# nvidia-cosmos/cosmos-curate

Measured on NVIDIA H100. Metric: clips_per_sec, higher is better.
Workload: dtype f16

## Files before the change

### cosmos_curate_b200/csrc/gemm.cu

```cuda
#include <cuda_fp16.h>

#include <algorithm>
#include <cstdlib>

#include "common.h"
#include "ptx.cuh"

namespace cb {

constexpr int BM = 128, BK = 64;
constexpr int kGemmThreads = 384;
constexpr int kEpiRows = 64, kEpiBytes = kEpiRows * 128;

template <int BN>
struct GemmCfg {
  static constexpr int kStages = (BN == 256) ? 4 : 6;
  static constexpr int kABytes = BM * BK * 2, kBBytes = BN * BK * 2;
  static constexpr int kStageBytes = kABytes + kBBytes;
  static constexpr int kRingBytes = kStages * kStageBytes;
  static constexpr int kEpiTotal = 2  * 2  * kEpiBytes;
  static constexpr int kSmem = kRingBytes + kEpiTotal + 1024  + 256 ;
  static_assert(kSmem <= 232448, "over the 227 KB of opt-in shared memory per block on sm_90");
};

struct GemmArgs {
  const float* bias;
  int M, N, K;
  int residual;
};

__device__ __forceinline__ float act_quick_gelu(float x) { return __fdividef(x, 1.f + exp2f(-2.4554669595930156f * x)); }
__device__ __forceinline__ float act_gelu_tanh(float x) {
  const float k0 = 0.7978845608028654f, k1 = 0.044715f;
  const float u = k0 * (x + k1 * x * x * x);
  const float e = exp2f(2.885390081777927f * u);
  const float t = 1.f - __fdividef(2.f, e + 1.f);
  return 0.5f * x * (1.f + t);
}

template <int ACT>
__device__ __forceinline__ float act(float x) {
  if (ACT == CB_EPI_QUICK_GELU) return act_quick_gelu(x);
  if (ACT == CB_EPI_GELU_TANH) return act_gelu_tanh(x);
  return x;
}

template <int BN>
__device__ __forceinline__ void wgmma_tile(float* d, uint64_t da, uint64_t db, int accumulate) {
  if (BN == 256) wgmma_m64n256k16(d, da, db, accumulate);
  else wgmma_m64n128k16(d, da, db, accumulate);
}

template <int BN, int ACT, bool OUT_F32>
__global__ void __launch_bounds__(kGemmThreads, 1)
    gemm_wgmma_kernel(const __grid_constant__ CUtensorMap map_a, const __grid_constant__ CUtensorMap map_b, const __grid_constant__ CUtensorMap map_o,
                      const __grid_constant__ CUtensorMap map_r, const GemmArgs g) {
  using Cfg = GemmCfg<BN>;
  constexpr int kSliceCols = OUT_F32 ? 32 : 64;
  constexpr int kSlices = BN / kSliceCols;
  constexpr int kSliceJ = kSliceCols / 8;
  extern __shared__ __align__(1024) uint8_t smem_raw[];
  const uint32_t base = (smem_u32(smem_raw) + 1023u) & ~1023u;
  uint8_t* smem = smem_raw + (base - smem_u32(smem_raw));
  uint8_t* sA = smem;
  uint8_t* sB = smem + Cfg::kStages * Cfg::kABytes;
  uint8_t* sE = smem + Cfg::kRingBytes;
  uint64_t* full = (uint64_t*)(smem + Cfg::kRingBytes + Cfg::kEpiTotal);
  uint64_t* empty = full + Cfg::kStages;
  uint64_t* rfull = empty + Cfg::kStages;

  const int warp = threadIdx.x >> 5, lane = threadIdx.x & 31, wg = warp >> 2;
  const int m_tiles = (g.M + BM - 1) / BM, n_tiles = (g.N + BN - 1) / BN;
  const int num_tiles = m_tiles * n_tiles;
  const int num_kb = (g.K + BK - 1) / BK;
  const int first = blockIdx.x, step = gridDim.x;
  const bool has_res = OUT_F32 && g.residual;

  if (threadIdx.x == 0) {
    tma_prefetch_desc(&map_a);
    tma_prefetch_desc(&map_b);
    tma_prefetch_desc(&map_o);
    if (has_res) tma_prefetch_desc(&map_r);
    for (int i = 0; i < Cfg::kStages; ++i) {
      mbar_init(&full[i], 1);
      mbar_init(&empty[i], 2);
    }
    for (int i = 0; i < 4; ++i) mbar_init(&rfull[i], 1);
    fence_barrier_init();
  }
  __syncthreads();

  if (wg == 0) {
    reg_dealloc<40>();
    if (warp == 0 && lane == 0) {
      int stage = 0;
      uint32_t phase = 0;
      for (int t = first; t < num_tiles; t += step) {
        const int m_blk = t / n_tiles, n_blk = t % n_tiles;
        if (has_res)
          for (int r = 0; r < BM; r += kEpiRows)
            for (int cc = 0; cc < BN && n_blk * BN + cc < g.N; cc += kSliceCols) tma_prefetch_l2_2d(&map_r, n_blk * BN + cc, m_blk * BM + r);
        for (int kb = 0; kb < num_kb; ++kb) {
          mbar_wait(&empty[stage], phase ^ 1);
          mbar_expect_tx(&full[stage], Cfg::kStageBytes);
          tma_load_2d(sA + stage * Cfg::kABytes, &map_a, &full[stage], kb * BK, m_blk * BM);
          tma_load_2d(sB + stage * Cfg::kBBytes, &map_b, &full[stage], kb * BK, n_blk * BN);
          if (++stage == Cfg::kStages) stage = 0, phase ^= 1;
        }
      }
    }
  } else {
    reg_alloc<232>();
    const int c = wg - 1;
    const bool leader = (threadIdx.x & 127) == 0;
    auto release = [&](int s) {
      if (leader) mbar_arrive(&empty[s]);
    };
    uint8_t* ebuf = sE + c * 2 * kEpiBytes;
    uint64_t* rbar = rfull + 2 * c;
    int eb = 0;
    uint32_t rphase = 0;
    int stage = 0;
    uint32_t phase = 0;
    float acc[BN / 2];
    float2 bias[BN / 8];
    for (int t = first; t < num_tiles; t += step) {
      const int m_blk = t / n_tiles, n_blk = t % n_tiles;
      const int row0 = m_blk * BM + c * 64, col0 = n_blk * BN;
      const int nslices = row0 >= g.M ? 0 : std::min(kSlices, (g.N - col0 + kSliceCols - 1) / kSliceCols);
      int prev = -1;
      for (int kb = 0; kb < num_kb; ++kb) {
        mbar_wait(&full[stage], phase);
        const uint64_t da = wgmma_desc_sw128(smem_u32(sA + stage * Cfg::kABytes + c * (64 * 128)));
        const uint64_t db = wgmma_desc_sw128(smem_u32(sB + stage * Cfg::kBBytes));
        wgmma_fence();
#pragma unroll
        for (int k = 0; k < BK / 16; ++k) wgmma_tile<BN>(acc, da + (uint64_t)(2 * k), db + (uint64_t)(2 * k), (kb | k) != 0);
        wgmma_commit();
        if (kb == 0 && has_res && leader) {
          bulk_wait_read<0>();
          for (int s = 0; s < 2 && s < nslices; ++s) {
            const int b = eb ^ s;
            mbar_expect_tx(&rbar[b], kEpiBytes);
            tma_load_2d(ebuf + b * kEpiBytes, &map_r, &rbar[b], col0 + s * kSliceCols, row0);
          }
        }
        wgmma_wait<1>();
        if (prev >= 0) release(prev);
        prev = stage;
        if (++stage == Cfg::kStages) stage = 0, phase ^= 1;
      }
#pragma unroll
      for (int j = 0; j < BN / 8; ++j) {
        const int col = col0 + 8 * j + 2 * (lane & 3);
        bias[j] = (g.bias && col < g.N) ? __ldg((const float2*)(g.bias + col)) : make_float2(0.f, 0.f);
      }
      wgmma_wait<0>();
      release(prev);

      const int rl = (warp & 3) * 16 + (lane >> 2), sw = lane >> 2;
#pragma unroll
      for (int s = 0; s < kSlices; ++s) {
        if (s >= nslices) break;
        uint8_t* buf = ebuf + eb * kEpiBytes;
        if (has_res) {
          mbar_wait(&rbar[eb], (rphase >> eb) & 1);
          rphase ^= 1u << eb;
        } else {
          if (leader) bulk_wait_read<1>();
          named_bar_sync(1 + c, 128);
        }
#pragma unroll
        for (int jj = 0; jj < kSliceJ; ++jj) {
          const int j = s * kSliceJ + jj;
#pragma unroll
          for (int h = 0; h < 2; ++h) {
            uint8_t* row = buf + (rl + 8 * h) * 128;
            float v0 = act<ACT>(acc[4 * j + 2 * h] + bias[j].x), v1 = act<ACT>(acc[4 * j + 2 * h + 1] + bias[j].y);
            if (OUT_F32) {
              float2* p = (float2*)(row + (((2 * jj + ((lane & 3) >> 1)) ^ sw) << 4) + 8 * (lane & 1));
              if (has_res) {
                const float2 rr = *p;
                v0 += rr.x, v1 += rr.y;
              }
              *p = make_float2(v0, v1);
            } else {
              *(__half2*)(row + ((jj ^ sw) << 4) + 4 * (lane & 3)) = __floats2half2_rn(v0, v1);
            }
          }
        }
        fence_proxy_async();
        named_bar_sync(1 + c, 128);
        if (leader) {
          tma_store_2d(&map_o, buf, col0 + s * kSliceCols, row0);
          bulk_commit();
          if (has_res && s + 2 < nslices) {
            bulk_wait_read<0>();
            mbar_expect_tx(&rbar[eb], kEpiBytes);
            tma_load_2d(buf, &map_r, &rbar[eb], col0 + (s + 2) * kSliceCols, row0);
          }
        }
        eb ^= 1;
      }
    }
    if (leader) bulk_wait<0>();
  }
}

template <int BN, int ACT, bool OUT_F32>
static int launch_gemm(cb_ctx* ctx, const CUtensorMap& ma, const CUtensorMap& mb, const CUtensorMap& mo, const CUtensorMap& mr, const GemmArgs& g,
                       cudaStream_t stream) {
  using Cfg = GemmCfg<BN>;
  auto kern = gemm_wgmma_kernel<BN, ACT, OUT_F32>;
  static bool attr_done[64] = {};
  bool& attr_set = attr_done[ctx->device & 63];
  if (!attr_set) {
    CB_CUDA(ctx, cudaFuncSetAttribute(kern, cudaFuncAttributeMaxDynamicSharedMemorySize, Cfg::kSmem));
    attr_set = true;
  }
  const int tiles = ((g.M + BM - 1) / BM) * ((g.N + BN - 1) / BN);
  mark_launch(ctx, CB_PROF_GEMM, stream);
  kern<<<std::min(tiles, ctx->sm_count), kGemmThreads, Cfg::kSmem, stream>>>(ma, mb, mo, mr, g);
  CB_CUDA(ctx, cudaGetLastError());
  return CB_OK;
}

template <int BN>
static int dispatch_gemm(cb_ctx* ctx, const CUtensorMap& ma, const CUtensorMap& mb, const CUtensorMap& mo, const CUtensorMap& mr, const GemmArgs& g,
                         bool out_f32, int epilogue, cudaStream_t stream) {
  if (out_f32) return launch_gemm<BN, CB_EPI_NONE, true>(ctx, ma, mb, mo, mr, g, stream);
  if (epilogue == CB_EPI_QUICK_GELU) return launch_gemm<BN, CB_EPI_QUICK_GELU, false>(ctx, ma, mb, mo, mr, g, stream);
  if (epilogue == CB_EPI_GELU_TANH) return launch_gemm<BN, CB_EPI_GELU_TANH, false>(ctx, ma, mb, mo, mr, g, stream);
  if (epilogue == CB_EPI_NONE) return launch_gemm<BN, CB_EPI_NONE, false>(ctx, ma, mb, mo, mr, g, stream);
  return fail(ctx, CB_ERR_ARG, "gemm: unknown epilogue %d", epilogue);
}

int gemm_f16(cb_ctx* ctx, const void* A, const void* W, const float* bias, const float* residual, float* out_f32, void* out_f16, int M,
             int N, int K, int epilogue, cudaStream_t stream) {
  if (!A || !W || (!out_f32 && !out_f16)) return fail(ctx, CB_ERR_ARG, "gemm: null operand");
  if (M <= 0 || N <= 0 || K <= 0) return fail(ctx, CB_ERR_ARG, "gemm: bad shape %dx%dx%d", M, N, K);
  if ((K & 7) || (N & 7)) return fail(ctx, CB_ERR_ARG, "gemm: N and K must be multiples of 8 (got N=%d K=%d)", N, K);
  if (((uintptr_t)A | (uintptr_t)W) & 15) return fail(ctx, CB_ERR_ARG, "gemm: operands must be 16-byte aligned");
  const void* out = out_f32 ? (const void*)out_f32 : out_f16;
  if (((uintptr_t)out | (uintptr_t)residual) & 15) return fail(ctx, CB_ERR_ARG, "gemm: output and residual must be 16-byte aligned");
  if (out_f32 && epilogue != CB_EPI_NONE) return fail(ctx, CB_ERR_UNSUPPORTED, "gemm: activation with fp32 output");
  if (residual && !out_f32) return fail(ctx, CB_ERR_UNSUPPORTED, "gemm: residual needs the fp32 output");
  const int tiles256 = ((M + BM - 1) / BM) * ((N + 255) / 256);
  const bool wide = (N % 256 == 0 || N > 1024) && tiles256 >= ctx->sm_count;
  const int BN = wide ? 256 : 128;
  CUtensorMap ma, mb, mo, mr;
  uint64_t da[2] = {(uint64_t)K, (uint64_t)M}, db[2] = {(uint64_t)K, (uint64_t)N}, st[1] = {(uint64_t)K * 2};
  uint32_t ba[2] = {BK, BM}, bb[2] = {BK, (uint32_t)BN};
  int rc = make_tensor_map(ctx, &ma, CU_TENSOR_MAP_DATA_TYPE_FLOAT16, 2, A, da, st, ba, CU_TENSOR_MAP_SWIZZLE_128B);
  if (rc) return rc;
  rc = make_tensor_map(ctx, &mb, CU_TENSOR_MAP_DATA_TYPE_FLOAT16, 2, W, db, st, bb, CU_TENSOR_MAP_SWIZZLE_128B);
  if (rc) return rc;
  const uint64_t esz = out_f32 ? 4 : 2;
  uint64_t dout[2] = {(uint64_t)N, (uint64_t)M}, sout[1] = {(uint64_t)N * esz};
  uint32_t bout[2] = {(uint32_t)(128 / esz), (uint32_t)kEpiRows};
  const CUtensorMapDataType dt = out_f32 ? CU_TENSOR_MAP_DATA_TYPE_FLOAT32 : CU_TENSOR_MAP_DATA_TYPE_FLOAT16;
  rc = make_tensor_map(ctx, &mo, dt, 2, out, dout, sout, bout, CU_TENSOR_MAP_SWIZZLE_128B);
  if (rc) return rc;
  mr = mo;
  if (residual && (rc = make_tensor_map(ctx, &mr, dt, 2, residual, dout, sout, bout, CU_TENSOR_MAP_SWIZZLE_128B))) return rc;
  GemmArgs g{bias, M, N, K, residual != nullptr};
  return BN == 256 ? dispatch_gemm<256>(ctx, ma, mb, mo, mr, g, out_f32 != nullptr, epilogue, stream)
                   : dispatch_gemm<128>(ctx, ma, mb, mo, mr, g, out_f32 != nullptr, epilogue, stream);
}

}

extern "C" int cb_gemm_f16(cb_ctx* ctx, const void* A, const void* W, const float* bias, const float* residual, float* out_f32,
                           void* out_f16, int M, int N, int K, int epilogue, void* stream) {
  if (!ctx) return CB_ERR_ARG;
  return cb::gemm_f16(ctx, A, W, bias, residual, out_f32, out_f16, M, N, K, epilogue, (cudaStream_t)stream);
}
```

### cosmos_curate_b200/csrc/ptx.cuh

```cuda
#pragma once
#include <cuda.h>
#include <cuda_fp16.h>
#include <stdint.h>

namespace cb {

__device__ __forceinline__ uint32_t smem_u32(const void* p) { return (uint32_t)__cvta_generic_to_shared(p); }

__device__ __forceinline__ void mbar_init(uint64_t* bar, uint32_t count) {
  asm volatile("mbarrier.init.shared::cta.b64 [%0], %1;" ::"r"(smem_u32(bar)), "r"(count));
}
__device__ __forceinline__ void fence_barrier_init() { asm volatile("fence.mbarrier_init.release.cluster;" ::: "memory"); }
__device__ __forceinline__ void fence_proxy_async() { asm volatile("fence.proxy.async.shared::cta;" ::: "memory"); }
__device__ __forceinline__ void mbar_expect_tx(uint64_t* bar, uint32_t bytes) {
  asm volatile("mbarrier.arrive.expect_tx.shared::cta.b64 _, [%0], %1;" ::"r"(smem_u32(bar)), "r"(bytes) : "memory");
}
__device__ __forceinline__ void mbar_arrive(uint64_t* bar) {
  asm volatile("mbarrier.arrive.shared::cta.b64 _, [%0];" ::"r"(smem_u32(bar)) : "memory");
}
__device__ __forceinline__ bool mbar_try_wait(uint64_t* bar, uint32_t parity) {
  uint32_t ok;
  asm volatile(
      "{\n\t.reg .pred p;\n\t"
      "mbarrier.try_wait.parity.shared::cta.b64 p, [%1], %2;\n\t"
      "selp.u32 %0, 1, 0, p;\n\t}"
      : "=r"(ok)
      : "r"(smem_u32(bar)), "r"(parity)
      : "memory");
  return ok != 0;
}
__device__ __forceinline__ void mbar_wait(uint64_t* bar, uint32_t parity) {
  while (!mbar_try_wait(bar, parity)) {
  }
}
__device__ __forceinline__ bool mbar_test(uint64_t* bar, uint32_t parity) {
  uint32_t ok;
  asm volatile(
      "{\n\t.reg .pred p;\n\t"
      "mbarrier.test_wait.parity.shared::cta.b64 p, [%1], %2;\n\t"
      "selp.u32 %0, 1, 0, p;\n\t}"
      : "=r"(ok)
      : "r"(smem_u32(bar)), "r"(parity)
      : "memory");
  return ok != 0;
}
__device__ __forceinline__ void mbar_wait_parked(uint64_t* bar, uint32_t parity, uint32_t ns = 20000) {
  uint32_t ok;
  do {
    asm volatile(
        "{\n\t.reg .pred p;\n\t"
        "mbarrier.try_wait.parity.shared::cta.b64 p, [%1], %2, %3;\n\t"
        "selp.u32 %0, 1, 0, p;\n\t}"
        : "=r"(ok)
        : "r"(smem_u32(bar)), "r"(parity), "r"(ns)
        : "memory");
  } while (!ok);
}

__device__ __forceinline__ void tma_prefetch_desc(const CUtensorMap* m) {
  asm volatile("prefetch.tensormap [%0];" ::"l"(m) : "memory");
}
__device__ __forceinline__ void tma_load_2d(void* dst, const CUtensorMap* m, uint64_t* bar, int c0, int c1) {
  asm volatile(
      "cp.async.bulk.tensor.2d.shared::cluster.global.mbarrier::complete_tx::bytes [%0], [%1, {%3, %4}], [%2];" ::"r"(smem_u32(dst)),
      "l"(m), "r"(smem_u32(bar)), "r"(c0), "r"(c1)
      : "memory");
}
__device__ __forceinline__ void tma_load_3d(void* dst, const CUtensorMap* m, uint64_t* bar, int c0, int c1, int c2) {
  asm volatile(
      "cp.async.bulk.tensor.3d.shared::cluster.global.mbarrier::complete_tx::bytes [%0], [%1, {%3, %4, %5}], [%2];" ::"r"(
          smem_u32(dst)),
      "l"(m), "r"(smem_u32(bar)), "r"(c0), "r"(c1), "r"(c2)
      : "memory");
}
__device__ __forceinline__ void tma_load_2d_hint(void* dst, const CUtensorMap* m, uint64_t* bar, int c0, int c1, uint64_t policy) {
  asm volatile(
      "cp.async.bulk.tensor.2d.shared::cluster.global.mbarrier::complete_tx::bytes.L2::cache_hint [%0], [%1, {%3, %4}], [%2], %5;" ::"r"(
          smem_u32(dst)),
      "l"(m), "r"(smem_u32(bar)), "r"(c0), "r"(c1), "l"(policy)
      : "memory");
}
__device__ __forceinline__ void tma_prefetch_l2_2d(const CUtensorMap* m, int c0, int c1) {
  asm volatile("cp.async.bulk.prefetch.tensor.2d.L2.global.tile [%0, {%1, %2}];" ::"l"(m), "r"(c0), "r"(c1) : "memory");
}

__device__ __forceinline__ void tma_store_2d(const CUtensorMap* m, const void* src, int c0, int c1) {
  asm volatile("cp.async.bulk.tensor.2d.global.shared::cta.bulk_group [%0, {%2, %3}], [%1];" ::"l"(m), "r"(smem_u32(src)), "r"(c0), "r"(c1)
               : "memory");
}
__device__ __forceinline__ void bulk_commit() { asm volatile("cp.async.bulk.commit_group;" ::: "memory"); }
template <int N>
__device__ __forceinline__ void bulk_wait_read() {
  asm volatile("cp.async.bulk.wait_group.read %0;" ::"n"(N) : "memory");
}
template <int N>
__device__ __forceinline__ void bulk_wait() {
  asm volatile("cp.async.bulk.wait_group %0;" ::"n"(N) : "memory");
}
__device__ __forceinline__ void named_bar_sync(int id, int threads) { asm volatile("bar.sync %0, %1;" ::"r"(id), "r"(threads) : "memory"); }

__device__ __forceinline__ uint64_t policy_evict_first() {
  uint64_t p;
  asm volatile("createpolicy.fractional.L2::evict_first.b64 %0, 1.0;" : "=l"(p));
  return p;
}
__device__ __forceinline__ uint64_t policy_evict_last() {
  uint64_t p;
  asm volatile("createpolicy.fractional.L2::evict_last.b64 %0, 1.0;" : "=l"(p));
  return p;
}
__device__ __forceinline__ void wgmma_fence() { asm volatile("wgmma.fence.sync.aligned;" ::: "memory"); }
__device__ __forceinline__ void wgmma_commit() { asm volatile("wgmma.commit_group.sync.aligned;" ::: "memory"); }
template <int N>
__device__ __forceinline__ void wgmma_wait() {
  asm volatile("wgmma.wait_group.sync.aligned %0;" ::"n"(N) : "memory");
}
template <int REGS>
__device__ __forceinline__ void reg_alloc() { asm volatile("setmaxnreg.inc.sync.aligned.u32 %0;" ::"n"(REGS)); }
template <int REGS>
__device__ __forceinline__ void reg_dealloc() { asm volatile("setmaxnreg.dec.sync.aligned.u32 %0;" ::"n"(REGS)); }

__device__ __forceinline__ uint64_t wgmma_desc_sw128(uint32_t smem_addr) {
  return (uint64_t)((smem_addr & 0x3FFFF) >> 4) | ((uint64_t)1 << 16) | ((uint64_t)(1024 >> 4) << 32) | ((uint64_t)1 << 62);
}
__device__ __forceinline__ uint64_t wgmma_desc_sw128_mn(uint32_t smem_addr) {
  return (uint64_t)((smem_addr & 0x3FFFF) >> 4) | ((uint64_t)(1024 >> 4) << 16) | ((uint64_t)(1024 >> 4) << 32) | ((uint64_t)1 << 62);
}

__device__ __forceinline__ void wgmma_m64n8k16(float* d, uint64_t desc_a, uint64_t desc_b, int accumulate) {
  asm volatile(
      "{\n\t.reg .pred p;\n\tsetp.ne.b32 p, %6, 0;\n\t"
      "wgmma.mma_async.sync.aligned.m64n8k16.f32.f16.f16 {%0, %1, %2, %3}, %4, %5, p, 1, 1, 0, 0;\n\t}"
      :
        "+f"(d[0]), "+f"(d[1]), "+f"(d[2]), "+f"(d[3])
      : "l"(desc_a), "l"(desc_b), "r"(accumulate));
}
__device__ __forceinline__ void wgmma_m64n32k16(float* d, uint64_t desc_a, uint64_t desc_b, int accumulate) {
  asm volatile(
      "{\n\t.reg .pred p;\n\tsetp.ne.b32 p, %18, 0;\n\t"
      "wgmma.mma_async.sync.aligned.m64n32k16.f32.f16.f16 {%0, %1, %2, %3, %4, %5, %6, %7, %8, %9, %10, %11, %12, %13, %14, %15}, %16, %17, p, 1, 1, 0, 0;\n\t}"
      :
        "+f"(d[0]), "+f"(d[1]), "+f"(d[2]), "+f"(d[3]), "+f"(d[4]), "+f"(d[5]), "+f"(d[6]), "+f"(d[7]),
        "+f"(d[8]), "+f"(d[9]), "+f"(d[10]), "+f"(d[11]), "+f"(d[12]), "+f"(d[13]), "+f"(d[14]), "+f"(d[15])
      : "l"(desc_a), "l"(desc_b), "r"(accumulate));
}
__device__ __forceinline__ void wgmma_m64n128k16(float* d, uint64_t desc_a, uint64_t desc_b, int accumulate) {
  asm volatile(
      "{\n\t.reg .pred p;\n\tsetp.ne.b32 p, %66, 0;\n\t"
      "wgmma.mma_async.sync.aligned.m64n128k16.f32.f16.f16 {%0, %1, %2, %3, %4, %5, %6, %7, %8, %9, %10, %11, %12, %13, %14, %15, %16, %17, %18, %19, %20, %21, %22, %23, %24, %25, %26, %27, %28, %29, %30, %31, %32, %33, %34, %35, %36, %37, %38, %39, %40, %41, %42, %43, %44, %45, %46, %47, %48, %49, %50, %51, %52, %53, %54, %55, %56, %57, %58, %59, %60, %61, %62, %63}, %64, %65, p, 1, 1, 0, 0;\n\t}"
      :
        "+f"(d[0]), "+f"(d[1]), "+f"(d[2]), "+f"(d[3]), "+f"(d[4]), "+f"(d[5]), "+f"(d[6]), "+f"(d[7]),
        "+f"(d[8]), "+f"(d[9]), "+f"(d[10]), "+f"(d[11]), "+f"(d[12]), "+f"(d[13]), "+f"(d[14]), "+f"(d[15]),
        "+f"(d[16]), "+f"(d[17]), "+f"(d[18]), "+f"(d[19]), "+f"(d[20]), "+f"(d[21]), "+f"(d[22]), "+f"(d[23]),
        "+f"(d[24]), "+f"(d[25]), "+f"(d[26]), "+f"(d[27]), "+f"(d[28]), "+f"(d[29]), "+f"(d[30]), "+f"(d[31]),
        "+f"(d[32]), "+f"(d[33]), "+f"(d[34]), "+f"(d[35]), "+f"(d[36]), "+f"(d[37]), "+f"(d[38]), "+f"(d[39]),
        "+f"(d[40]), "+f"(d[41]), "+f"(d[42]), "+f"(d[43]), "+f"(d[44]), "+f"(d[45]), "+f"(d[46]), "+f"(d[47]),
        "+f"(d[48]), "+f"(d[49]), "+f"(d[50]), "+f"(d[51]), "+f"(d[52]), "+f"(d[53]), "+f"(d[54]), "+f"(d[55]),
        "+f"(d[56]), "+f"(d[57]), "+f"(d[58]), "+f"(d[59]), "+f"(d[60]), "+f"(d[61]), "+f"(d[62]), "+f"(d[63])
      : "l"(desc_a), "l"(desc_b), "r"(accumulate));
}
__device__ __forceinline__ void wgmma_m64n256k16(float* d, uint64_t desc_a, uint64_t desc_b, int accumulate) {
  asm volatile(
      "{\n\t.reg .pred p;\n\tsetp.ne.b32 p, %130, 0;\n\t"
      "wgmma.mma_async.sync.aligned.m64n256k16.f32.f16.f16 {%0, %1, %2, %3, %4, %5, %6, %7, %8, %9, %10, %11, %12, %13, %14, %15, %16, %17, %18, %19, %20, %21, %22, %23, %24, %25, %26, %27, %28, %29, %30, %31, %32, %33, %34, %35, %36, %37, %38, %39, %40, %41, %42, %43, %44, %45, %46, %47, %48, %49, %50, %51, %52, %53, %54, %55, %56, %57, %58, %59, %60, %61, %62, %63, %64, %65, %66, %67, %68, %69, %70, %71, %72, %73, %74, %75, %76, %77, %78, %79, %80, %81, %82, %83, %84, %85, %86, %87, %88, %89, %90, %91, %92, %93, %94, %95, %96, %97, %98, %99, %100, %101, %102, %103, %104, %105, %106, %107, %108, %109, %110, %111, %112, %113, %114, %115, %116, %117, %118, %119, %120, %121, %122, %123, %124, %125, %126, %127}, %128, %129, p, 1, 1, 0, 0;\n\t}"
      :
        "+f"(d[0]), "+f"(d[1]), "+f"(d[2]), "+f"(d[3]), "+f"(d[4]), "+f"(d[5]), "+f"(d[6]), "+f"(d[7]),
        "+f"(d[8]), "+f"(d[9]), "+f"(d[10]), "+f"(d[11]), "+f"(d[12]), "+f"(d[13]), "+f"(d[14]), "+f"(d[15]),
        "+f"(d[16]), "+f"(d[17]), "+f"(d[18]), "+f"(d[19]), "+f"(d[20]), "+f"(d[21]), "+f"(d[22]), "+f"(d[23]),
        "+f"(d[24]), "+f"(d[25]), "+f"(d[26]), "+f"(d[27]), "+f"(d[28]), "+f"(d[29]), "+f"(d[30]), "+f"(d[31]),
        "+f"(d[32]), "+f"(d[33]), "+f"(d[34]), "+f"(d[35]), "+f"(d[36]), "+f"(d[37]), "+f"(d[38]), "+f"(d[39]),
        "+f"(d[40]), "+f"(d[41]), "+f"(d[42]), "+f"(d[43]), "+f"(d[44]), "+f"(d[45]), "+f"(d[46]), "+f"(d[47]),
        "+f"(d[48]), "+f"(d[49]), "+f"(d[50]), "+f"(d[51]), "+f"(d[52]), "+f"(d[53]), "+f"(d[54]), "+f"(d[55]),
        "+f"(d[56]), "+f"(d[57]), "+f"(d[58]), "+f"(d[59]), "+f"(d[60]), "+f"(d[61]), "+f"(d[62]), "+f"(d[63]),
        "+f"(d[64]), "+f"(d[65]), "+f"(d[66]), "+f"(d[67]), "+f"(d[68]), "+f"(d[69]), "+f"(d[70]), "+f"(d[71]),
        "+f"(d[72]), "+f"(d[73]), "+f"(d[74]), "+f"(d[75]), "+f"(d[76]), "+f"(d[77]), "+f"(d[78]), "+f"(d[79]),
        "+f"(d[80]), "+f"(d[81]), "+f"(d[82]), "+f"(d[83]), "+f"(d[84]), "+f"(d[85]), "+f"(d[86]), "+f"(d[87]),
        "+f"(d[88]), "+f"(d[89]), "+f"(d[90]), "+f"(d[91]), "+f"(d[92]), "+f"(d[93]), "+f"(d[94]), "+f"(d[95]),
        "+f"(d[96]), "+f"(d[97]), "+f"(d[98]), "+f"(d[99]), "+f"(d[100]), "+f"(d[101]), "+f"(d[102]), "+f"(d[103]),
        "+f"(d[104]), "+f"(d[105]), "+f"(d[106]), "+f"(d[107]), "+f"(d[108]), "+f"(d[109]), "+f"(d[110]), "+f"(d[111]),
        "+f"(d[112]), "+f"(d[113]), "+f"(d[114]), "+f"(d[115]), "+f"(d[116]), "+f"(d[117]), "+f"(d[118]), "+f"(d[119]),
        "+f"(d[120]), "+f"(d[121]), "+f"(d[122]), "+f"(d[123]), "+f"(d[124]), "+f"(d[125]), "+f"(d[126]), "+f"(d[127])
      : "l"(desc_a), "l"(desc_b), "r"(accumulate));
}
__device__ __forceinline__ void wgmma_m64n64k16_ra_tb(float* d, const uint32_t* a, uint64_t desc_b, int accumulate) {
  asm volatile(
      "{\n\t.reg .pred p;\n\tsetp.ne.b32 p, %37, 0;\n\t"
      "wgmma.mma_async.sync.aligned.m64n64k16.f32.f16.f16 {%0, %1, %2, %3, %4, %5, %6, %7, %8, %9, %10, %11, %12, %13, %14, %15, %16, %17, %18, %19, %20, %21, %22, %23, %24, %25, %26, %27, %28, %29, %30, %31}, {%32, %33, %34, %35}, %36, p, 1, 1, 1;\n\t}"
      :
        "+f"(d[0]), "+f"(d[1]), "+f"(d[2]), "+f"(d[3]), "+f"(d[4]), "+f"(d[5]), "+f"(d[6]), "+f"(d[7]),
        "+f"(d[8]), "+f"(d[9]), "+f"(d[10]), "+f"(d[11]), "+f"(d[12]), "+f"(d[13]), "+f"(d[14]), "+f"(d[15]),
        "+f"(d[16]), "+f"(d[17]), "+f"(d[18]), "+f"(d[19]), "+f"(d[20]), "+f"(d[21]), "+f"(d[22]), "+f"(d[23]),
        "+f"(d[24]), "+f"(d[25]), "+f"(d[26]), "+f"(d[27]), "+f"(d[28]), "+f"(d[29]), "+f"(d[30]), "+f"(d[31])
      : "r"(a[0]), "r"(a[1]), "r"(a[2]), "r"(a[3]), "l"(desc_b), "r"(accumulate));
}

__device__ __forceinline__ uint32_t cluster_ctarank() {
  uint32_t r;
  asm volatile("mov.u32 %0, %%cluster_ctarank;" : "=r"(r));
  return r;
}
__device__ __forceinline__ void cluster_sync_all() {
  asm volatile("barrier.cluster.arrive.release.aligned;" ::: "memory");
  asm volatile("barrier.cluster.wait.acquire.aligned;" ::: "memory");
}
__device__ __forceinline__ void mbar_arrive_cluster(uint32_t addr) {
  asm volatile("mbarrier.arrive.release.cluster.shared::cluster.b64 _, [%0];" ::"r"(addr) : "memory");
}
__device__ __forceinline__ uint32_t map_to_cta(const void* local, uint32_t rank) {
  uint32_t r;
  asm volatile("mapa.shared::cluster.u32 %0, %1, %2;" : "=r"(r) : "r"(smem_u32(local)), "r"(rank));
  return r;
}

}
```

Measured before the change: 250.8.

## Add ping-pong warpgroup GEMM schedule for large tiles with heavy epilogues

Adds a ping-pong mode where each consumer warpgroup computes a whole 128x128 tile and the two warpgroups alternate tiles. Named barriers hand off the mainloop turn so one group's epilogue (activation or residual add) overlaps the other's MMAs. It is chosen for large GEMMs with N divisible by 256 that carry an activation or residual. The residual L2 prefetch moves from the producer to the consumer leaders, and the stage count is now derived from the shared-memory limit. Each ping-pong warpgroup holds twice as many accumulator registers, which raises register pressure, and the barrier handoff ordering is delicate.

Result: faster. 258.1, median of 6 (+2.9%).

```diff
diff --git a/cosmos_curate_b200/csrc/gemm.cu b/cosmos_curate_b200/csrc/gemm.cu
--- a/cosmos_curate_b200/csrc/gemm.cu
+++ b/cosmos_curate_b200/csrc/gemm.cu
@@ -8,19 +8,22 @@
 
 namespace cb {
 
-constexpr int BM = 128, BK = 64;
+constexpr int BK = 64;
 constexpr int kGemmThreads = 384;
 constexpr int kEpiRows = 64, kEpiBytes = kEpiRows * 128;
+constexpr int kSmemLimit = 232448;
+constexpr int BM = 128;
+constexpr int kBarTurn = 3;
 
 template <int BN>
 struct GemmCfg {
-  static constexpr int kStages = (BN == 256) ? 4 : 6;
   static constexpr int kABytes = BM * BK * 2, kBBytes = BN * BK * 2;
   static constexpr int kStageBytes = kABytes + kBBytes;
+  static constexpr int kEpiTotal = 2  * 2  * kEpiBytes;
+  static constexpr int kStages = std::min(6, (kSmemLimit - kEpiTotal - 1024 - 256) / kStageBytes);
   static constexpr int kRingBytes = kStages * kStageBytes;
-  static constexpr int kEpiTotal = 2  * 2  * kEpiBytes;
   static constexpr int kSmem = kRingBytes + kEpiTotal + 1024  + 256 ;
-  static_assert(kSmem <= 232448, "over the 227 KB of opt-in shared memory per block on sm_90");
+  static_assert(kSmem <= kSmemLimit, "over the opt-in shared memory per block");
 };
 
 struct GemmArgs {
@@ -51,11 +54,14 @@
   else wgmma_m64n128k16(d, da, db, accumulate);
 }
 
-template <int BN, int ACT, bool OUT_F32>
+template <int WM, int BN, bool PP, int ACT, bool OUT_F32>
 __global__ void __launch_bounds__(kGemmThreads, 1)
     gemm_wgmma_kernel(const __grid_constant__ CUtensorMap map_a, const __grid_constant__ CUtensorMap map_b, const __grid_constant__ CUtensorMap map_o,
                       const __grid_constant__ CUtensorMap map_r, const GemmArgs g) {
   using Cfg = GemmCfg<BN>;
+  static_assert(WM * (PP ? 1 : 2) == BM, "a ping-pong warpgroup computes the whole tile, a cooperative one half of it");
+  constexpr int kBlocks = WM / 64;
+  constexpr int kAcc = BN / 2;
   constexpr int kSliceCols = OUT_F32 ? 32 : 64;
   constexpr int kSlices = BN / kSliceCols;
   constexpr int kSliceJ = kSliceCols / 8;
@@ -83,7 +89,7 @@
     if (has_res) tma_prefetch_desc(&map_r);
     for (int i = 0; i < Cfg::kStages; ++i) {
       mbar_init(&full[i], 1);
-      mbar_init(&empty[i], 2);
+      mbar_init(&empty[i], PP ? 1 : 2);
     }
     for (int i = 0; i < 4; ++i) mbar_init(&rfull[i], 1);
     fence_barrier_init();
@@ -97,9 +103,6 @@
       uint32_t phase = 0;
       for (int t = first; t < num_tiles; t += step) {
         const int m_blk = t / n_tiles, n_blk = t % n_tiles;
-        if (has_res)
-          for (int r = 0; r < BM; r += kEpiRows)
-            for (int cc = 0; cc < BN && n_blk * BN + cc < g.N; cc += kSliceCols) tma_prefetch_l2_2d(&map_r, n_blk * BN + cc, m_blk * BM + r);
         for (int kb = 0; kb < num_kb; ++kb) {
           mbar_wait(&empty[stage], phase ^ 1);
           mbar_expect_tx(&full[stage], Cfg::kStageBytes);
@@ -120,30 +123,43 @@
     uint64_t* rbar = rfull + 2 * c;
     int eb = 0;
     uint32_t rphase = 0;
-    int stage = 0;
-    uint32_t phase = 0;
-    float acc[BN / 2];
+    float acc[kBlocks * kAcc];
     float2 bias[BN / 8];
-    for (int t = first; t < num_tiles; t += step) {
+    constexpr int kTileStep = PP ? 2 : 1;
+    for (int i = PP ? c : 0, t = first + i * step; t < num_tiles; i += kTileStep, t += kTileStep * step) {
       const int m_blk = t / n_tiles, n_blk = t % n_tiles;
-      const int row0 = m_blk * BM + c * 64, col0 = n_blk * BN;
-      const int nslices = row0 >= g.M ? 0 : std::min(kSlices, (g.N - col0 + kSliceCols - 1) / kSliceCols);
+      const int row_in_tile = PP ? 0 : c * WM;
+      const int row0 = m_blk * BM + row_in_tile, col0 = n_blk * BN;
+      const int nb = row0 >= g.M ? 0 : std::min(kBlocks, (g.M - row0 + 63) / 64);
+      const int ns = std::min(kSlices, (g.N - col0 + kSliceCols - 1) / kSliceCols);
+      const int nq = nb * ns;
+      auto load_residual = [&](int q, int b) {
+        const int blk = q / ns;
+        mbar_expect_tx(&rbar[b], kEpiBytes);
+        tma_load_2d(ebuf + b * kEpiBytes, &map_r, &rbar[b], col0 + (q - blk * ns) * kSliceCols, row0 + 64 * blk);
+      };
+      if (has_res && leader)
+        for (int q = 0; q < nq; ++q) tma_prefetch_l2_2d(&map_r, col0 + (q % ns) * kSliceCols, row0 + 64 * (q / ns));
+
+      int stage = (i * num_kb) % Cfg::kStages;
+      uint32_t phase = ((i * num_kb) / Cfg::kStages) & 1;
+      if (PP && i > 0) named_bar_sync(kBarTurn + c, 256);
       int prev = -1;
       for (int kb = 0; kb < num_kb; ++kb) {
         mbar_wait(&full[stage], phase);
-        const uint64_t da = wgmma_desc_sw128(smem_u32(sA + stage * Cfg::kABytes + c * (64 * 128)));
+        const uint64_t da = wgmma_desc_sw128(smem_u32(sA + stage * Cfg::kABytes + row_in_tile * 128));
         const uint64_t db = wgmma_desc_sw128(smem_u32(sB + stage * Cfg::kBBytes));
         wgmma_fence();
 #pragma unroll
-        for (int k = 0; k < BK / 16; ++k) wgmma_tile<BN>(acc, da + (uint64_t)(2 * k), db + (uint64_t)(2 * k), (kb | k) != 0);
+        for (int k = 0; k < BK / 16; ++k)
+#pragma unroll
+          for (int blk = 0; blk < kBlocks; ++blk)
+            wgmma_tile<BN>(acc + blk * kAcc, da + (uint64_t)(blk * (64 * 128 >> 4) + 2 * k), db + (uint64_t)(2 * k), (kb | k) != 0);
         wgmma_commit();
+        if (PP && kb == num_kb - 1 && t + step < num_tiles) named_bar_arrive(kBarTurn + (c ^ 1), 256);
         if (kb == 0 && has_res && leader) {
           bulk_wait_read<0>();
-          for (int s = 0; s < 2 && s < nslices; ++s) {
-            const int b = eb ^ s;
-            mbar_expect_tx(&rbar[b], kEpiBytes);
-            tma_load_2d(ebuf + b * kEpiBytes, &map_r, &rbar[b], col0 + s * kSliceCols, row0);
-          }
+          for (int q = 0; q < 2 && q < nq; ++q) load_residual(q, eb ^ q);
         }
         wgmma_wait<1>();
         if (prev >= 0) release(prev);
@@ -159,59 +175,64 @@
       release(prev);
 
       const int rl = (warp & 3) * 16 + (lane >> 2), sw = lane >> 2;
-#pragma unroll
-      for (int s = 0; s < kSlices; ++s) {
-        if (s >= nslices) break;
-        uint8_t* buf = ebuf + eb * kEpiBytes;
-        if (has_res) {
-          mbar_wait(&rbar[eb], (rphase >> eb) & 1);
-          rphase ^= 1u << eb;
-        } else {
-          if (leader) bulk_wait_read<1>();
-          named_bar_sync(1 + c, 128);
-        }
-#pragma unroll
-        for (int jj = 0; jj < kSliceJ; ++jj) {
-          const int j = s * kSliceJ + jj;
-#pragma unroll
-          for (int h = 0; h < 2; ++h) {
-            uint8_t* row = buf + (rl + 8 * h) * 128;
-            float v0 = act<ACT>(acc[4 * j + 2 * h] + bias[j].x), v1 = act<ACT>(acc[4 * j + 2 * h + 1] + bias[j].y);
-            if (OUT_F32) {
-              float2* p = (float2*)(row + (((2 * jj + ((lane & 3) >> 1)) ^ sw) << 4) + 8 * (lane & 1));
-              if (has_res) {
-                const float2 rr = *p;
-                v0 += rr.x, v1 += rr.y;
+      int q = 0;
+#pragma unroll
+      for (int blk = 0; blk < kBlocks; ++blk) {
+#pragma unroll
+        for (int s = 0; s < kSlices; ++s) {
+          if (blk >= nb || s >= ns) break;
+          uint8_t* buf = ebuf + eb * kEpiBytes;
+          if (has_res) {
+            mbar_wait(&rbar[eb], (rphase >> eb) & 1);
+            rphase ^= 1u << eb;
+          } else {
+            if (leader) bulk_wait_read<1>();
+            named_bar_sync(1 + c, 128);
+          }
+#pragma unroll
+          for (int jj = 0; jj < kSliceJ; ++jj) {
+            const int j = s * kSliceJ + jj;
+            const float* a = acc + blk * kAcc + 4 * j;
+#pragma unroll
+            for (int h = 0; h < 2; ++h) {
+              uint8_t* row = buf + (rl + 8 * h) * 128;
+              float v0 = act<ACT>(a[2 * h] + bias[j].x), v1 = act<ACT>(a[2 * h + 1] + bias[j].y);
+              if (OUT_F32) {
+                float2* p = (float2*)(row + (((2 * jj + ((lane & 3) >> 1)) ^ sw) << 4) + 8 * (lane & 1));
+                if (has_res) {
+                  const float2 rr = *p;
+                  v0 += rr.x, v1 += rr.y;
+                }
+                *p = make_float2(v0, v1);
+              } else {
+                *(__half2*)(row + ((jj ^ sw) << 4) + 4 * (lane & 3)) = __floats2half2_rn(v0, v1);
               }
-              *p = make_float2(v0, v1);
-            } else {
-              *(__half2*)(row + ((jj ^ sw) << 4) + 4 * (lane & 3)) = __floats2half2_rn(v0, v1);
             }
           }
+          fence_proxy_async();
+          named_bar_sync(1 + c, 128);
+          if (leader) {
+            tma_store_2d(&map_o, buf, col0 + s * kSliceCols, row0 + 64 * blk);
+            bulk_commit();
+            if (has_res && q + 2 < nq) {
+              bulk_wait_read<0>();
+              load_residual(q + 2, eb);
+            }
+          }
+          eb ^= 1;
+          ++q;
         }
-        fence_proxy_async();
-        named_bar_sync(1 + c, 128);
-        if (leader) {
-          tma_store_2d(&map_o, buf, col0 + s * kSliceCols, row0);
-          bulk_commit();
-          if (has_res && s + 2 < nslices) {
-            bulk_wait_read<0>();
-            mbar_expect_tx(&rbar[eb], kEpiBytes);
-            tma_load_2d(buf, &map_r, &rbar[eb], col0 + (s + 2) * kSliceCols, row0);
-          }
-        }
-        eb ^= 1;
       }
     }
     if (leader) bulk_wait<0>();
   }
 }
 
-template <int BN, int ACT, bool OUT_F32>
+template <int WM, int BN, bool PP, int ACT, bool OUT_F32>
 static int launch_gemm(cb_ctx* ctx, const CUtensorMap& ma, const CUtensorMap& mb, const CUtensorMap& mo, const CUtensorMap& mr, const GemmArgs& g,
                        cudaStream_t stream) {
   using Cfg = GemmCfg<BN>;
-  auto kern = gemm_wgmma_kernel<BN, ACT, OUT_F32>;
+  auto kern = gemm_wgmma_kernel<WM, BN, PP, ACT, OUT_F32>;
   static bool attr_done[64] = {};
   bool& attr_set = attr_done[ctx->device & 63];
   if (!attr_set) {
@@ -225,13 +246,13 @@
   return CB_OK;
 }
 
-template <int BN>
+template <int WM, int BN, bool PP>
 static int dispatch_gemm(cb_ctx* ctx, const CUtensorMap& ma, const CUtensorMap& mb, const CUtensorMap& mo, const CUtensorMap& mr, const GemmArgs& g,
                          bool out_f32, int epilogue, cudaStream_t stream) {
-  if (out_f32) return launch_gemm<BN, CB_EPI_NONE, true>(ctx, ma, mb, mo, mr, g, stream);
-  if (epilogue == CB_EPI_QUICK_GELU) return launch_gemm<BN, CB_EPI_QUICK_GELU, false>(ctx, ma, mb, mo, mr, g, stream);
-  if (epilogue == CB_EPI_GELU_TANH) return launch_gemm<BN, CB_EPI_GELU_TANH, false>(ctx, ma, mb, mo, mr, g, stream);
-  if (epilogue == CB_EPI_NONE) return launch_gemm<BN, CB_EPI_NONE, false>(ctx, ma, mb, mo, mr, g, stream);
+  if (out_f32) return launch_gemm<WM, BN, PP, CB_EPI_NONE, true>(ctx, ma, mb, mo, mr, g, stream);
+  if (epilogue == CB_EPI_QUICK_GELU) return launch_gemm<WM, BN, PP, CB_EPI_QUICK_GELU, false>(ctx, ma, mb, mo, mr, g, stream);
+  if (epilogue == CB_EPI_GELU_TANH) return launch_gemm<WM, BN, PP, CB_EPI_GELU_TANH, false>(ctx, ma, mb, mo, mr, g, stream);
+  if (epilogue == CB_EPI_NONE) return launch_gemm<WM, BN, PP, CB_EPI_NONE, false>(ctx, ma, mb, mo, mr, g, stream);
   return fail(ctx, CB_ERR_ARG, "gemm: unknown epilogue %d", epilogue);
 }
 
@@ -246,7 +267,9 @@
   if (out_f32 && epilogue != CB_EPI_NONE) return fail(ctx, CB_ERR_UNSUPPORTED, "gemm: activation with fp32 output");
   if (residual && !out_f32) return fail(ctx, CB_ERR_UNSUPPORTED, "gemm: residual needs the fp32 output");
   const int tiles256 = ((M + BM - 1) / BM) * ((N + 255) / 256);
-  const bool wide = (N % 256 == 0 || N > 1024) && tiles256 >= ctx->sm_count;
+  const bool large = (N % 256 == 0 || N > 1024) && tiles256 >= ctx->sm_count;
+  const bool pingpong = large && N % 256 == 0 && (residual || epilogue != CB_EPI_NONE);
+  const bool wide = large && !pingpong;
   const int BN = wide ? 256 : 128;
   CUtensorMap ma, mb, mo, mr;
   uint64_t da[2] = {(uint64_t)K, (uint64_t)M}, db[2] = {(uint64_t)K, (uint64_t)N}, st[1] = {(uint64_t)K * 2};
@@ -264,8 +287,10 @@
   mr = mo;
   if (residual && (rc = make_tensor_map(ctx, &mr, dt, 2, residual, dout, sout, bout, CU_TENSOR_MAP_SWIZZLE_128B))) return rc;
   GemmArgs g{bias, M, N, K, residual != nullptr};
-  return BN == 256 ? dispatch_gemm<256>(ctx, ma, mb, mo, mr, g, out_f32 != nullptr, epilogue, stream)
-                   : dispatch_gemm<128>(ctx, ma, mb, mo, mr, g, out_f32 != nullptr, epilogue, stream);
+  const bool f32 = out_f32 != nullptr;
+  if (pingpong) return dispatch_gemm<128, 128, true>(ctx, ma, mb, mo, mr, g, f32, epilogue, stream);
+  if (wide) return dispatch_gemm<64, 256, false>(ctx, ma, mb, mo, mr, g, f32, epilogue, stream);
+  return dispatch_gemm<64, 128, false>(ctx, ma, mb, mo, mr, g, f32, epilogue, stream);
 }
 
 }
diff --git a/cosmos_curate_b200/csrc/ptx.cuh b/cosmos_curate_b200/csrc/ptx.cuh
--- a/cosmos_curate_b200/csrc/ptx.cuh
+++ b/cosmos_curate_b200/csrc/ptx.cuh
@@ -98,6 +98,7 @@
   asm volatile("cp.async.bulk.wait_group %0;" ::"n"(N) : "memory");
 }
 __device__ __forceinline__ void named_bar_sync(int id, int threads) { asm volatile("bar.sync %0, %1;" ::"r"(id), "r"(threads) : "memory"); }
+__device__ __forceinline__ void named_bar_arrive(int id, int threads) { asm volatile("bar.arrive %0, %1;" ::"r"(id), "r"(threads) : "memory"); }
 
 __device__ __forceinline__ uint64_t policy_evict_first() {
   uint64_t p;
```
